# TrevorS/qwen3-tts-rs

Hardware: AMD Instinct MI355X
Metric: acoustic_frames_per_sec (higher is better)
Workload: dtype bf16

## Files before the change

### qwen3_tts_rs_amd/csrc/q3_codec_run.hip

```cpp
#include "q3_engine.h"

namespace {
struct DevCache {
    std::mutex mu;
    std::unordered_multimap<uint64_t, void*> free_blocks;
    std::unordered_map<void*, uint64_t> live;
    size_t cached = 0, cap = 0;
    DevCache() { const char* e = getenv("Q3_DEV_CACHE_MB"); cap = (size_t)(e ? atol(e) : 32768) << 20; }
    static uint64_t key(int dev, size_t bytes) { return ((uint64_t)dev << 48) | (uint64_t)bytes; }
    static size_t size_class(size_t bytes) {
        if (bytes <= 4096) return (bytes + 255) & ~(size_t)255;
        size_t p2 = 1; while ((p2 << 1) <= bytes) p2 <<= 1;
        const size_t step = p2 >> 4;
        return (bytes + step - 1) / step * step;
    }
    hipError_t get(void** p, size_t bytes) {
        bytes = size_class(bytes);
        int dev = 0; (void)hipGetDevice(&dev);
        const uint64_t k = key(dev, bytes);
        {
            std::lock_guard<std::mutex> g(mu);
            auto it = free_blocks.find(k);
            if (it != free_blocks.end()) { *p = it->second; free_blocks.erase(it); cached -= bytes; live[*p] = k; return hipSuccess; }
        }
// ... 86 lines not shown
static thread_local const q3_model* tl_codec_model = nullptr;
static const void* packed_of(const float* w) { return tl_codec_model ? tl_codec_model->pk(w) : nullptr; }
static thread_local int tl_codec_planes = 3;
CodecScope::CodecScope(const q3_model* m) {
    static const int env_planes = [] { const char* e = getenv("Q3_CODEC_PLANES"); const int v = e ? atoi(e) : 0; return (v == 2 || v == 3) ? v : 0; }();
    planes = env_planes ? env_planes : m->codec_planes;
    tl_codec_model = m; tl_codec_planes = planes;
}
CodecScope::~CodecScope() { tl_codec_planes = 3; }
static hipError_t conv1(const float* x, const float* w, const float* b, float* y, int cin, int cout, int L, hipStream_t st,
                        const float* resid = nullptr, const float* scale = nullptr, int act = 0,
                        const float* sa = nullptr, const float* sib = nullptr) {
    ConvArgs a; a.x = x; a.w = w; a.b = b; a.y = y; a.cin = cin; a.cout = cout; a.L = L; a.k = 1; a.dil = 1;
    a.resid = resid; a.scale = scale; a.act = act; a.snake_a = sa; a.snake_b = sib; a.wpk = packed_of(w); a.planes = tl_codec_planes;
    return launch_conv1d(a, st);
}
static hipError_t convk(const float* x, const float* w, const float* b, float* y, int cin, int cout, int L, int k, int dil,
                        hipStream_t st, const float* sa = nullptr, const float* sib = nullptr, int act = 0) {
    ConvArgs a; a.x = x; a.w = w; a.b = b; a.y = y; a.cin = cin; a.cout = cout; a.L = L; a.k = k; a.dil = dil;
    a.snake_a = sa; a.snake_b = sib; a.act = act; a.wpk = packed_of(w); a.planes = tl_codec_planes;
    return launch_conv1d(a, st);
}

static q3_status tap_out(float** taps, int id, const float* dev, size_t n, hipStream_t st) {
    if (taps && taps[id]) { HIPC(hipStreamSynchronize(st)); HIPC(q3_hipMemcpy(taps[id], dev, n * 4, hipMemcpyDeviceToHost)); }
    return Q3_OK;
}
q3_status codec_front_quant(const q3_model* m, CodecWS& ws, int T, hipStream_t st) {
    const q3_config& c = m->cfg;
    const int CD = c.dec_cb_dim, Q = c.dec_q_dim;
    float *A = ws.bufA, *B = ws.bufB;
    float* e1 = A; float* e2 = A + (size_t)CD * T;
    HIPC(launch_rvq_embed(ws.frames, T, m->first_cb, m->rest_cbs_dev, e1, e2, CD, c.dec_cb_size, st));
    HIPC(conv1(e1, m->first_proj, nullptr, B, CD, Q, T, st));
    HIPC(conv1(e2, m->rest_proj, nullptr, B, CD, Q, T, st, B));
    return Q3_OK;
}
q3_status codec_front_preconv(const q3_model* m, const float* x, float* y, int L, hipStream_t st) {
    HIPC(convk(x, m->pre_w, m->pre_b, y, m->cfg.dec_q_dim, m->cfg.dec_latent, L, 3, 1, st));
    return Q3_OK;
}
q3_status codec_front_transformer(const q3_model* m, CodecWS& ws, int T, hipStream_t st, const CodecAttnFn& rope_attn) {
    const q3_config& c = m->cfg;
    const int LAT = c.dec_latent, DH = c.dec_hidden, QD = c.dec_heads * c.dec_head_dim, DI = c.dec_inter;
    float *A = ws.bufA, *B = ws.bufB, *C = ws.bufC, *D = ws.bufD, *E = ws.bufE;
    float* Hd = D;
    HIPC(conv1(C, m->inp_w, m->inp_b, Hd, LAT, DH, T, st));
    float* Nn = E;
    float* q = A; float* k = A + (size_t)QD * T; float* v = A + (size_t)2 * QD * T; float* ao = A + (size_t)3 * QD * T;
    float* g = B; float* u = B + (size_t)DI * T;
    for (int l = 0; l < c.dec_layers; ++l) {
        const DecLayerW& L = m->dl[l];
        HIPC(launch_rmsnorm_c(Hd, L.in_ln, Nn, DH, T, c.dec_eps, st));
        auto adjacent = [&](const float* w0, const float* w1, int cout, int cin) {
            const char* p0 = (const char*)m->pk(w0); const char* p1 = (const char*)m->pk(w1);
            return p0 && p1 && p1 == p0 + packed_conv_w_bytes(cout, cin, 1) && w1 == w0 + (size_t)cout * cin &&
                   cout % 32 == 0 && cin % 16 == 0;
        };
        static const bool no_fuse_qkv = getenv("Q3_CODEC_NO_QKV_FUSE") != nullptr || getenv("Q3_CONV_F32") != nullptr ||
                                        getenv("Q3_CONV_VALU") != nullptr;
        if (!no_fuse_qkv && adjacent(L.q, L.k, QD, DH) && adjacent(L.k, L.v, QD, DH)) {
            HIPC(conv1(Nn, L.q, nullptr, q, DH, 3 * QD, T, st));
        } else {
            HIPC(conv1(Nn, L.q, nullptr, q, DH, QD, T, st));
            HIPC(conv1(Nn, L.k, nullptr, k, DH, QD, T, st));
            HIPC(conv1(Nn, L.v, nullptr, v, DH, QD, T, st));
        }
        Q3C(rope_attn(l, q, k, v, ao));
        HIPC(conv1(ao, L.o, nullptr, Hd, QD, DH, T, st, Hd, L.attn_scale));
        HIPC(launch_rmsnorm_c(Hd, L.post_ln, Nn, DH, T, c.dec_eps, st));
        if (!no_fuse_qkv && adjacent(L.gate, L.up, DI, DH)) {
            HIPC(conv1(Nn, L.gate, nullptr, g, DH, 2 * DI, T, st));
        } else {
            HIPC(conv1(Nn, L.gate, nullptr, g, DH, DI, T, st));
            HIPC(conv1(Nn, L.up, nullptr, u, DH, DI, T, st));
        }
        HIPC(launch_silu_mul(g, u, g, (int64_t)DI * T, st));
        HIPC(conv1(g, L.down, nullptr, Hd, DI, DH, T, st, Hd, L.mlp_scale));
    }
    HIPC(launch_rmsnorm_c(Hd, m->dec_norm, Nn, DH, T, c.dec_eps, st));
    HIPC(conv1(Nn, m->outp_w, m->outp_b, C, DH, LAT, T, st));
    return Q3_OK;
}
q3_status codec_stack_dev(const q3_model* m, CodecWS& ws, float* cur, int L, hipStream_t st, float** taps, const CodecScope& scope) {
    const int NPL = scope.planes;
    const q3_config& c = m->cfg;
    const int LAT = c.dec_latent;
    auto TAP = [&](int id, const float* dev, size_t n) -> q3_status { return tap_out(taps, id, dev, n, st); };
    float *A = ws.bufA, *B = ws.bufB, *C = ws.bufC;
    for (int i = 0; i < 2; ++i) {
        const UpW& U = m->up[i];
        float* upo = (cur == C) ? A : C;
        HIPC(launch_transconv1d_taps(cur, U.tw, U.tb, upo, LAT, LAT, L, U.ratio, 1, nullptr, nullptr, st, nullptr, nullptr, nullptr, m->pk(U.tw), NPL));
        L *= U.ratio;
        float* dw = (upo == A) ? C : A;
        HIPC(launch_dwconv7(upo, U.dww, U.dwb, dw, LAT, L, st));
        float* ln = dw + (size_t)LAT * L;
        HIPC(launch_layernorm_c(dw, U.nw, U.nb, ln, LAT, L, 1e-6f, st));
        HIPC(conv1(ln, U.p1w, U.p1b, B, LAT, 4 * LAT, L, st, nullptr, nullptr, 1));
        HIPC(conv1(B, U.p2w, U.p2b, upo, 4 * LAT, LAT, L, st, upo, U.gamma));
        cur = upo;
        Q3C(TAP(Q3_DEC_UP0 + i, cur, (size_t)LAT * L));
    }
    int Cc = c.dec_dim;
    float* pool4[4] = {A, B, C, ws.bufF};
    auto other = [&](std::initializer_list<const float*> used) -> float* {
        for (float* p : pool4) { bool u = false; for (const float* q : used) if (q == p) u = true; if (!u) return p; }
        return nullptr;
    };
    float* xact = other({cur});
    {
        ConvArgs a; a.x = cur; a.w = m->init_w; a.wpk = m->pk(m->init_w); a.b = m->init_b; a.cin = LAT; a.cout = Cc; a.L = L; a.k = 7; a.dil = 1; a.planes = NPL;
        a.post_a = m->blk[0].a; a.post_ib = m->blk[0].ib;
        if (taps && taps[Q3_DEC_INIT]) { float* raw = other({cur, xact}); a.y = raw; a.y2 = xact; HIPC(launch_conv1d(a, st)); Q3C(TAP(Q3_DEC_INIT, raw, (size_t)Cc * L)); }
        else { a.y = xact; HIPC(launch_conv1d(a, st)); }
    }
    static const int dils[3] = {1, 3, 9};
    for (int b = 0; b < 4; ++b) {
        const DecBlockW& Bk = m->blk[b];
        float* Y = other({xact});
        float* YA = other({xact, Y});
        HIPC(launch_transconv1d_taps(xact, Bk.tw, Bk.tb, Y, Bk.cin, Bk.cout, L, Bk.rate, 2, nullptr, nullptr, st, Bk.res[0].a1, Bk.res[0].ib1, YA, m->pk(Bk.tw), NPL));
        L *= Bk.rate; Cc = Bk.cout;
        float* T2 = other({Y, YA});
        for (int uu = 0; uu < 3; ++uu) {
            const ResUnitW& R = Bk.res[uu];
            const float* nxt_a = uu < 2 ? Bk.res[uu + 1].a1 : (b < 3 ? m->blk[b + 1].a : m->fin_a);
            const float* nxt_ib = uu < 2 ? Bk.res[uu + 1].ib1 : (b < 3 ? m->blk[b + 1].ib : m->fin_ib);
            {
                ResUnitArgs r{};
                r.xa = YA; r.y = Y; r.ya = T2; r.w1pk = m->pk(R.c1w); r.w2pk = m->pk(R.c2w); r.b1 = R.c1b; r.b2 = R.c2b;
                r.mid_a = R.a2; r.mid_ib = R.ib2; r.post_a = nxt_a; r.post_ib = nxt_ib; r.C = Cc; r.L = L; r.dil = dils[uu]; r.planes = NPL;
                const hipError_t e = launch_resunit(r, st);
                if (e == hipSuccess) { float* t = YA; YA = T2; T2 = t; continue; }
                if (e != hipErrorNotSupported) HIPC(e);
            }
            {
                ConvArgs a; a.x = YA; a.w = R.c1w; a.wpk = m->pk(R.c1w); a.b = R.c1b; a.y = T2; a.cin = Cc; a.cout = Cc; a.L = L; a.k = 7; a.dil = dils[uu]; a.planes = NPL;
                a.post_a = R.a2; a.post_ib = R.ib2;
                HIPC(launch_conv1d(a, st));
            }
            {
                ConvArgs a; a.x = T2; a.w = R.c2w; a.wpk = m->pk(R.c2w); a.b = R.c2b; a.y = Y; a.y2 = YA; a.cin = Cc; a.cout = Cc; a.L = L; a.k = 1; a.dil = 1; a.resid = Y; a.planes = NPL;
                if (uu < 2) { a.post_a = Bk.res[uu + 1].a1; a.post_ib = Bk.res[uu + 1].ib1; }
                else if (b < 3) { a.post_a = m->blk[b + 1].a; a.post_ib = m->blk[b + 1].ib; }
                else { a.post_a = m->fin_a; a.post_ib = m->fin_ib; }
                HIPC(launch_conv1d(a, st));
            }
        }
        Q3C(TAP(Q3_DEC_BLK0 + b, Y, (size_t)Cc * L));
        xact = YA;
    }
    HIPC(convk(xact, m->fin_w, m->fin_b, ws.pcm, Cc, 1, L, 7, 1, st, nullptr, nullptr, 2));
    return Q3_OK;
}

q3_status codec_decode_dev(const q3_model* m, CodecWS& ws, int T, hipStream_t st, float** taps, int c0) {
    const q3_config& c = m->cfg;
    const CodecScope scope(m);
    const int Q = c.dec_q_dim, LAT = c.dec_latent;
    float *B = ws.bufB, *C = ws.bufC;
    Q3C(codec_front_quant(m, ws, T, st));
    Q3C(tap_out(taps, Q3_DEC_QUANT, B, (size_t)Q * T, st));
    Q3C(codec_front_preconv(m, B, C, T, st));
    Q3C(tap_out(taps, Q3_DEC_PRECONV, C, (size_t)LAT * T, st));
    const float scale = (float)pow((double)c.dec_head_dim, -0.5);
    Q3C(codec_front_transformer(m, ws, T, st, [&](int, float* q, float* k, float* v, float* ao) -> q3_status {
        HIPC(launch_rope_c(q, k, ws.cs, ws.sn, c.dec_heads, c.dec_head_dim, T, st));
        HIPC(launch_attn_c(q, k, v, ao, c.dec_heads, c.dec_head_dim, T, scale, st));
        return Q3_OK;
    }));
    Q3C(tap_out(taps, Q3_DEC_PRETRANS, C, (size_t)LAT * T, st));
    float* cur = C;
    int L = T;
    if (c0 > 0) {
        HIPC(launch_copy_rows(C + c0, T, ws.bufF, T - c0, LAT, T - c0, st));
        cur = ws.bufF; L = T - c0;
    }
    return codec_stack_dev(m, ws, cur, L, st, taps, scope);
}

extern "C" q3_status q3_decode_codes(q3_model* m, const uint32_t* frames_host, int n_frames, float* pcm_host, float** taps_host) {
    if (!m || !m->finalized) return set_err(Q3_INVALID_ARG, "model not finalized");
    if (n_frames < 0 || (n_frames > 0 && (!frames_host || !pcm_host))) return set_err(Q3_INVALID_ARG, "q3_decode_codes: bad argument");
    if (n_frames == 0) return Q3_OK;
    for (int f = 0; f < n_frames; ++f)
        for (int g = 1; g < 16; ++g)
            if (frames_host[(size_t)f * 16 + g] >= (uint32_t)m->cfg.dec_cb_size)
                return set_err(Q3_INVALID_ARG, "code %u out of range for codebook %d (frame %d)", frames_host[(size_t)f * 16 + g], g, f);
    HIPC(hipSetDevice(m->device));
    CodecWS ws;
    q3_status st = codec_reserve(m, ws, n_frames);
    if (st == Q3_OK) {
        hipError_t e = q3_hipMemcpy(ws.frames, frames_host, (size_t)n_frames * 16 * 4, hipMemcpyHostToDevice);
        if (e != hipSuccess) st = set_err(Q3_HIP_ERROR, "hipMemcpy frames: %s", hipGetErrorString(e));
    }
    if (st == Q3_OK) st = codec_decode_dev(m, ws, n_frames, 0, taps_host);
    if (st == Q3_OK) {
        hipError_t e = q3_hipDeviceSynchronize();
        if (e == hipSuccess) e = q3_hipMemcpy(pcm_host, ws.pcm, (size_t)n_frames * samples_per_frame(m->cfg) * 4, hipMemcpyDeviceToHost);
        if (e != hipSuccess) st = set_err(Q3_HIP_ERROR, "decode: %s", hipGetErrorString(e));
    }
    ws.release();
    return st;
}
```

### qwen3_tts_rs_amd/csrc/q3_engine.h

```cpp
#pragma once
#include "../../include/q3tts.h"
#include "q3_kernels.h"

#include <math.h>
#include <stdarg.h>
#include <stdio.h>
#include <string.h>

#include <algorithm>
#include <atomic>
#include <chrono>
#include <functional>
#include <memory>
#include <string>
#include <thread>
#include <mutex>
#include <unordered_map>
#include <vector>

#include "q3_internal.h"
#include "q3_aql.h"

using namespace q3;
#define Q3_HIDDEN __attribute__((visibility("hidden")))
// ... 225 lines not shown
    void release() {
        dev_free(bufA); dev_free(bufB); dev_free(bufC); dev_free(bufF); dev_free(bufD); dev_free(bufE); dev_free(cs); dev_free(sn); dev_free(frames); dev_free(pcm);
        bufA = bufB = bufC = bufF = bufD = bufE = cs = sn = pcm = nullptr; frames = nullptr; cap_frames = 0; cap_front = 0;
    }
};

struct LmBuf { float *X, *SUM, *QKV, *Q, *ATT, *ACT, *PART; };
struct LmDims { int H, I, nh, nkv, layers; float eps; };

struct BatReq {
    q3_request r{}; std::vector<uint32_t> text, instruct, ref_codes, ref_text; std::vector<float> xvec;
    void own(const q3_request& q, int hidden) {
        r = q;
        text.assign(q.text_ids, q.text_ids + (q.text_ids ? q.n_text : 0));
        instruct.assign(q.instruct_ids, q.instruct_ids + (q.instruct_ids ? q.n_instruct : 0));
        ref_codes.assign(q.ref_codes, q.ref_codes + (q.ref_codes ? (size_t)q.n_ref * 16 : 0));
        ref_text.assign(q.ref_text_ids, q.ref_text_ids + (q.ref_text_ids ? q.n_ref_text : 0));
        if (q.xvector) xvec.assign(q.xvector, q.xvector + hidden);
        fix();
    }
    void fix() {
        r.text_ids = text.empty() ? nullptr : text.data(); r.n_text = (int32_t)text.size();
        r.instruct_ids = instruct.empty() ? nullptr : instruct.data(); r.n_instruct = (int32_t)instruct.size();
        r.ref_codes = ref_codes.empty() ? nullptr : ref_codes.data(); r.n_ref = (int32_t)(ref_codes.size() / 16);
        r.ref_text_ids = ref_text.empty() ? nullptr : ref_text.data(); r.n_ref_text = (int32_t)ref_text.size();
        r.xvector = xvec.empty() ? nullptr : xvec.data();
    }
};
struct SeqInfo {
    q3_request req; std::vector<uint32_t> text, instruct, ref_codes, ref_text; std::vector<float> xvec; bool icl = false;
    int prefill_len = 0, trailing_len = 0, row_base = 0, n_rows = 0, trail_base = 0, pad_row = 0;
    int n_frames = 0; bool done = false;
    int start_run = 0, limit = 0, stream_pos = 0;
    int reused = 0;
    bool idle = false;
    int max_length_req = 0;
    bool opened = false, text_closed = true;
    std::vector<uint32_t> text_all;
    int n_trail = 0, ready = 0x7fffffff, committed = 0;
};

struct ProfAcc { double ms = 0; double bytes = 0; long launches = 0; };
struct ProfShape { int M, N, K, epi, rms, produce, tiled, count; };

struct q3_session {
    q3_model* m = nullptr; int B = 0;
    hipStream_t stream = nullptr; bool owns_stream = true;
    DevPool pool;
    std::vector<SeqInfo> seq;
    q3_options opts{};
    int max_frames = 0, max_seq = 0, prefill_len = 0, n_splits = 1;
    int* limit = nullptr;
    SampleRow* sample_rows = nullptr;
    int row_cap = 0, repl_base = 0;
    LmBuf tb{}, cb{};
    float *LASTH = nullptr, *LOGITS = nullptr, *CP_IN = nullptr, *CP_LOGITS = nullptr;
    float* wide_ws = nullptr; size_t wide_ws_bytes = 0;
    float *kcache = nullptr, *vcache = nullptr, *ckcache = nullptr, *cvcache = nullptr;
    size_t kv_layer_stride = 0, ckv_layer_stride = 0;
    bool paged = false; unsigned long long* kv_table = nullptr; std::vector<std::vector<float*>> kv_rows;
    std::vector<BatReq> ragged;
    bool regrouped = false;
    bool prefix_common = false;
    int kv_overflow_row = -1;
    bool kv_bf16 = false, kv_in_bf16 = false; unsigned long long* kv_conv = nullptr;
    float *rows = nullptr, *embeds = nullptr, *xvec = nullptr; int n_rows_total = 0;
    uint32_t* ids_dev = nullptr; int *tr_dev = nullptr, *ci_dev = nullptr; float *proj_e = nullptr, *proj_h = nullptr;
    uint32_t* ref_codes_dev = nullptr;
    int *trail_base = nullptr, *trail_len = nullptr, *pad_row = nullptr;
    int* text_ready = nullptr;
    uint32_t* app_ids = nullptr; float *app_e = nullptr, *app_h = nullptr, *app_out = nullptr;
    int* flush_buf = nullptr; size_t flush_cap = 0;
    uint32_t* tok = nullptr; uint8_t* seen = nullptr; int *frame_idx = nullptr, *pos = nullptr, *token_count = nullptr;
    float* U = nullptr; uint32_t* codes = nullptr;
    float* logits_hist = nullptr; float* cp_logits_hist = nullptr; bool debug = false;
    bool prefilled = false; int frames_run = 0;
    hipGraphExec_t graph_exec = nullptr; hipGraph_t graph = nullptr;
    q3::AqlProgram* aql = nullptr; int aql_mode = 0; bool aql_tried = false, aql_failed = false;
    bool precapture = false;
    CodecWS cws;
    q3_codec_stream* cstream = nullptr;
    hipStream_t dec_stream = nullptr; hipEvent_t dec_ev = nullptr;
    std::vector<CodecWS> par_ws; std::vector<hipStream_t> par_streams;
    CodecWS seg_ws;
    std::vector<uint32_t> codes_host; bool codes_host_valid = false;
    int stream_pos = 0;
    int stream_mode = 0;
    bool profile = false; ProfAcc prof_linear;
    bool legacy_attn = getenv("Q3_LEGACY_ATTN") != nullptr;
    bool proj_tables = getenv("Q3_NO_PROJ_TABLES") == nullptr;
    bool qkv_tables = getenv("Q3_NO_QKV_TABLES") == nullptr;
    bool ksplit = getenv("Q3_NO_KSPLIT") == nullptr;
    bool cp_attn = getenv("Q3_NO_CP_ATTN") == nullptr;
    bool no_chunk = getenv("Q3_NO_CHUNK") != nullptr;
    std::vector<std::pair<hipEvent_t, hipEvent_t>> prof_events; std::vector<double> prof_event_bytes;
    std::vector<hipEvent_t> prof_pool; size_t prof_pool_next = 0;
    std::vector<ProfShape> prof_shapes;
#ifdef Q3_TRACE
    unsigned long long* trace_buf = nullptr; int trace_node = 0, trace_cap = 0;
    struct TraceMeta { int kind, a, b, c, d, e, f; };
    std::vector<TraceMeta> trace_meta;
    unsigned long long* trace_next(int kind, int a, int b, int c, int d = 0, int e = 0, int f = 0) {
        if (!trace_buf || trace_node >= trace_cap) return nullptr;
        trace_meta.push_back({kind, a, b, c, d, e, f});
        return trace_buf + (size_t)(trace_node++) * TRACE_NODE;
    }
#endif
    ~q3_session();
};


Q3_HIDDEN void model_destroy(q3_model* m);
Q3_HIDDEN void retile_bf16(const uint16_t* src, int N, int K, uint16_t* dst, int mode);
Q3_HIDDEN q3_status codec_reserve(const q3_model* m, CodecWS& ws, int T, int Tf = 0);
Q3_HIDDEN int samples_per_frame(const q3_config& c);
Q3_HIDDEN q3_status codec_decode_dev(const q3_model* m, CodecWS& ws, int T, hipStream_t st, float** taps, int c0 = 0);
struct Q3_HIDDEN CodecScope { int planes; explicit CodecScope(const q3_model* m); ~CodecScope(); CodecScope(const CodecScope&) = delete; };
using CodecAttnFn = std::function<q3_status(int layer, float* q, float* k, float* v, float* ao)>;
Q3_HIDDEN q3_status codec_rope_table(const q3_config& c, int n, float* cs_dev, float* sn_dev);
Q3_HIDDEN q3_status codec_front_quant(const q3_model* m, CodecWS& ws, int T, hipStream_t st);
Q3_HIDDEN q3_status codec_front_preconv(const q3_model* m, const float* x, float* y, int L, hipStream_t st);
Q3_HIDDEN q3_status codec_front_transformer(const q3_model* m, CodecWS& ws, int T, hipStream_t st, const CodecAttnFn& rope_attn);
Q3_HIDDEN q3_status codec_stack_dev(const q3_model* m, CodecWS& ws, float* cur, int L, hipStream_t st, float** taps, const CodecScope& scope);
struct CsPush { int row; int n; int skip; const uint32_t* host; const uint32_t* dev; float* pcm_host; };
Q3_HIDDEN q3_status codec_stream_create(q3_model* m, int rows, int max_frames, hipStream_t st, q3_codec_stream** out, int block_frames = 0,
                                        int max_blocks = 0);
Q3_HIDDEN q3_status codec_stream_push(q3_codec_stream* cs, const std::vector<CsPush>& pushes);
Q3_HIDDEN int codec_stream_pos(const q3_codec_stream* cs, int row);
Q3_HIDDEN void codec_stream_blocks(const q3_codec_stream* cs, int row, int upto, int* held, int* need);
Q3_HIDDEN void codec_stream_reset(q3_codec_stream* cs, int row);
Q3_HIDDEN hipError_t sync_frames(q3_session* s);
Q3_HIDDEN q3_status kv_reserve_row(q3_session* s, int b, int n_pos);
Q3_HIDDEN q3_status kv_reserve_frames(q3_session* s, int frames);
Q3_HIDDEN void kv_release_row(q3_session* s, int b);
Q3_HIDDEN LmDims talker_dims(const q3_config& c);
Q3_HIDDEN LmDims cp_dims(const q3_config& c);
Q3_HIDDEN q3_status talker_step(q3_session* s, const int* pos_dev, int pos_static, bool with_head, int rows_per_seq = 1,
                                const int* text_ready = nullptr);
Q3_HIDDEN SampleRow sample_row(const q3_options& o);
Q3_HIDDEN void request_shape(const q3_request& r, int* prefill_len, int* limit);
Q3_HIDDEN long row_worst_units(int prefill_len, int limit, bool bf16);
Q3_HIDDEN q3_request idle_request(int chunk_frames);
Q3_HIDDEN q3_status session_create(q3_model* m, const q3_request* reqs, int batch, int frame_budget, int prompt_budget, q3_session** out,
                                   hipStream_t borrow = nullptr);
Q3_HIDDEN q3_status lm_layer(q3_session* s, const LmDims& d, const LayerW& w, LmBuf& b, float* kc, float* vc, int max_seq,
                             const int* pos_dev, int pos_static, int n_splits, int rows_per_seq = 1, bool skip_qkv = false,
                             const CpGatherArgs* fold = nullptr, int paged_layer = -1);
struct TextPiece { int b; const uint32_t* ids; int n; bool last; };
Q3_HIDDEN q3_status session_text_enable(q3_session* s);
Q3_HIDDEN q3_status session_append_many(q3_session* s, const std::vector<TextPiece>& pieces);
Q3_HIDDEN int session_row_remaining(const q3_session* s, int b);
Q3_HIDDEN int session_row_committed(const q3_session* s, int b);
Q3_HIDDEN q3_status transplant_row(q3_session* s, int b, q3_session* side, int j, int limit);
Q3_HIDDEN q3_status transplant_check(q3_session* s, q3_session* side, int j, int limit_req, int* limit_out);
```

### qwen3_tts_rs_amd/csrc/q3_session.hip

```cpp
#include "q3_engine.h"
#include "q3_prefix_cache.h"

hipError_t sync_frames(q3_session* s) {
    if (s->aql) {
        std::string why;
        if (!q3::aql_wait(s->aql, &why)) { s->aql_failed = true; set_err(Q3_HIP_ERROR, "AQL frame submission: %s", why.c_str()); return hipErrorUnknown; }
    }
    return hipStreamSynchronize(s->stream);
}

static hipError_t run_linear(q3_session* s, const LinArgs& a_in) {
    LinArgs a = a_in;
    a.ws = s->wide_ws; a.ws_bytes = s->wide_ws_bytes;
#ifdef Q3_TRACE
    a.trace = s->trace_next(0, a.M, a.N, a.K, a.epi, a.norm_w ? 1 : 0, a.tiled);
#endif
    if (!s->profile) return launch_linear(a, s->stream);
    hipEvent_t e0, e1;
    if (s->prof_pool_next + 2 <= s->prof_pool.size()) { e0 = s->prof_pool[s->prof_pool_next++]; e1 = s->prof_pool[s->prof_pool_next++]; }
    else {
        hipError_t e = hipEventCreate(&e0); if (e != hipSuccess) return e;
        e = hipEventCreate(&e1); if (e != hipSuccess) return e;
        s->prof_pool.push_back(e0); s->prof_pool.push_back(e1); s->prof_pool_next = s->prof_pool.size();
    }
// ... 501 lines not shown
    HIPC(alloc_lm(s->tb, talker_dims(c), s->n_splits));
    HIPC(alloc_lm(s->cb, cp_dims(c), 1));
    if (B > 16) {
        size_t need = 0;
        auto upd = [&](int N, int K, int epi) { if (N % 128 == 0 && K % 128 == 0) { const size_t b = gemm_wide_ws_bytes(B, N, K, epi); if (b > need) need = b; } };
        const int QDt = c.n_heads * HEAD_DIM, KDt = c.n_kv_heads * HEAD_DIM, QDc = c.cp_heads * HEAD_DIM, KDc = c.cp_kv_heads * HEAD_DIM;
        upd(QDt + 2 * KDt, H, EPI_NONE); upd(H, QDt, EPI_RESID); upd(c.inter, H, EPI_SWIGLU); upd(H, c.inter, EPI_RESID); upd(c.codec_vocab, H, EPI_NONE);
        upd(QDc + 2 * KDc, c.cp_hidden, EPI_NONE); upd(c.cp_hidden, QDc, EPI_RESID); upd(c.cp_inter, c.cp_hidden, EPI_SWIGLU); upd(c.cp_hidden, c.cp_inter, EPI_RESID);
        upd(c.cp_vocab, c.cp_hidden, EPI_NONE); upd(c.cp_hidden, H, EPI_NONE);
        if (need) { HIPC(s->pool.alloc(&s->wide_ws, need / 4)); s->wide_ws_bytes = need; }
    }
    HIPC(s->pool.alloc(&s->LASTH, (size_t)B * H));
    HIPC(s->pool.alloc(&s->LOGITS, (size_t)B * c.codec_vocab));
    HIPC(s->pool.alloc(&s->CP_IN, (size_t)(B > 16 ? up16(B) : 16) * H));
    HIPC(s->pool.alloc(&s->CP_LOGITS, (size_t)15 * B * c.cp_vocab));
    s->kv_layer_stride = (size_t)B * c.n_kv_heads * s->max_seq * HEAD_DIM;
    {
        const char* e = getenv("Q3_KV_CONTIGUOUS");
        s->paged = !(e && atoi(e) != 0);
        if (s->paged) {
            if (s->max_seq > KV_MAX_PAGES * KV_PAGE_POS) return set_err(Q3_KV_OVERFLOW, "sequence length %d exceeds a row's page table (%d)", s->max_seq, KV_MAX_PAGES * KV_PAGE_POS);
            HIPC(s->pool.alloc(&s->kv_table, (size_t)B * KV_MAX_PAGES));
            HIPC(s->pool.alloc(&s->kv_conv, (size_t)2 * B * KV_MAX_PAGES));
            s->kv_rows.resize((size_t)B);
            for (auto& r : s->kv_rows) r.reserve(KV_MAX_PAGES);
        } else {
            HIPC(s->pool.alloc(&s->kcache, s->kv_layer_stride * c.n_layers));
            HIPC(s->pool.alloc(&s->vcache, s->kv_layer_stride * c.n_layers));
        }
    }
    s->ckv_layer_stride = (size_t)B * c.cp_kv_heads * (c.n_groups + 1) * HEAD_DIM;
    HIPC(s->pool.alloc(&s->ckcache, 2 * s->ckv_layer_stride * c.cp_layers + 64));
    s->cvcache = s->ckcache + s->ckv_layer_stride * c.cp_layers + 64;
    HIPC(s->pool.alloc(&s->rows, ((size_t)rows + (size_t)B * s->row_cap) * H));
    HIPC(s->pool.alloc(&s->limit, B));
    HIPC(s->pool.alloc(&s->sample_rows, B));
    {
        std::vector<int> lim(B); std::vector<SampleRow> sr(B);
        for (int b = 0; b < B; ++b) { lim[b] = s->seq[b].limit; sr[b] = sample_row(s->seq[b].req.opts); }
        HIPC(q3_hipMemcpy(s->limit, lim.data(), B * 4, hipMemcpyHostToDevice));
        HIPC(q3_hipMemcpy(s->sample_rows, sr.data(), B * sizeof(SampleRow), hipMemcpyHostToDevice));
    }
    HIPC(s->pool.alloc(&s->embeds, (size_t)B * s->prefill_len * H));
    HIPC(s->pool.alloc(&s->xvec, (size_t)B * H));
    HIPC(s->pool.alloc(&s->ids_dev, (size_t)rows)); HIPC(s->pool.alloc(&s->tr_dev, (size_t)B * s->prefill_len)); HIPC(s->pool.alloc(&s->ci_dev, (size_t)B * s->prefill_len));
    HIPC(s->pool.alloc(&s->proj_e, (size_t)rows * c.text_dim)); HIPC(s->pool.alloc(&s->proj_h, (size_t)rows * c.text_dim));
    HIPC(s->pool.alloc(&s->trail_base, B)); HIPC(s->pool.alloc(&s->trail_len, B)); HIPC(s->pool.alloc(&s->pad_row, B));
    HIPC(s->pool.alloc(&s->tok, B)); HIPC(s->pool.alloc(&s->seen, (size_t)B * c.codec_vocab));
    HIPC(s->pool.alloc(&s->frame_idx, B)); HIPC(s->pool.alloc(&s->pos, B)); HIPC(s->pool.alloc(&s->token_count, B));
    HIPC(s->pool.alloc(&s->U, (size_t)B * (s->max_frames + 2)));
    HIPC(s->pool.alloc(&s->codes, (size_t)B * s->max_frames * 16));
    std::vector<float> U((size_t)B * (s->max_frames + 2), 0.0f);
    for (int b = 0; b < B; ++b) {
        uint64_t st;
        const q3_options& o = reqs[b].opts;
        uint64_t seed = o.seed;
        if (!o.has_seed) seed = (uint64_t)std::chrono::high_resolution_clock::now().time_since_epoch().count() + 0x9E37ULL * b;
        q3_rng_seed(seed, &st);
        for (int i = 0; i <= s->max_frames; ++i) U[(size_t)b * (s->max_frames + 2) + i] = q3_rng_next(&st);
    }
    HIPC(q3_hipMemcpy(s->U, U.data(), U.size() * 4, hipMemcpyHostToDevice));
    HIPC(s->pool.settle());
    s->pool.lazy = false;
    *out = s.release();
    return Q3_OK;
}

q3_session::~q3_session() {
    if (!m) return;
    (void)hipSetDevice(m->device);
    if (stream) (void)hipStreamSynchronize(stream);
    if (dec_stream) (void)hipStreamSynchronize(dec_stream);
    for (auto st : par_streams) (void)hipStreamSynchronize(st);
    if (aql) q3::aql_program_destroy(aql);
    for (int b = 0; b < (int)kv_rows.size(); ++b) kv_release_row(this, b);
    if (graph_exec) (void)hipGraphExecDestroy(graph_exec);
    if (graph) (void)hipGraphDestroy(graph);
    for (auto& ev : prof_pool) (void)hipEventDestroy(ev);
    for (auto st : par_streams) (void)hipStreamDestroy(st);
    if (cstream) q3_codec_stream_free(cstream);
    cws.release(); seg_ws.release();
    for (auto& w : par_ws) w.release();
    if (dec_ev) (void)hipEventDestroy(dec_ev);
    if (dec_stream) (void)hipStreamDestroy(dec_stream);
    if (stream && owns_stream) {
        std::lock_guard<std::mutex> g(m->stream_mu);
        if (m->idle_streams.size() < 16) { m->idle_streams.push_back(stream); stream = nullptr; }
    }
    if (stream && owns_stream) (void)hipStreamDestroy(stream);
    pool.release_all();
    if (m->refs.fetch_sub(1) == 1) model_destroy(m);
}

extern "C" void q3_session_free(q3_session* s) { delete s; }

extern "C" q3_status q3_session_set_kv_dtype(q3_session* s, int dtype) {
    if (!s) return set_err(Q3_INVALID_ARG, "null session");
    if (s->prefilled) return set_err(Q3_INVALID_ARG, "q3_session_set_kv_dtype must be called before prefill");
    if (dtype != Q3_DTYPE_F32 && dtype != Q3_DTYPE_BF16) return set_err(Q3_INVALID_ARG, "q3_session_set_kv_dtype: unknown dtype %d", dtype);
    if (dtype == Q3_DTYPE_BF16 && !s->paged) return set_err(Q3_UNSUPPORTED, "bf16 K/V needs the paged cache (Q3_KV_CONTIGUOUS is set)");
    s->kv_bf16 = dtype == Q3_DTYPE_BF16;
    return Q3_OK;
}

extern "C" q3_status q3_session_set_debug(q3_session* s, int capture) {
    if (!s) return set_err(Q3_INVALID_ARG, "null session");
    if (s->prefilled) return set_err(Q3_INVALID_ARG, "set_debug must be called before prefill");
    if (capture && s->text_ready) return set_err(Q3_UNSUPPORTED, "set_debug: the session has open text rows");
    s->debug = capture != 0;
    if (s->debug && !s->logits_hist) {
        const q3_config& c = s->m->cfg;
        HIPC(hipSetDevice(s->m->device));
        HIPC(s->pool.alloc(&s->logits_hist, (size_t)s->B * (s->max_frames + 1) * c.codec_vocab));
        HIPC(s->pool.alloc(&s->cp_logits_hist, (size_t)s->max_frames * 15 * s->B * c.cp_vocab));
    }
    return Q3_OK;
}
extern "C" q3_status q3_session_set_profile(q3_session* s, int enable) {
    if (!s) return set_err(Q3_INVALID_ARG, "null session");
    if (enable && s->text_ready) return set_err(Q3_UNSUPPORTED, "set_profile: the session has open text rows");
    s->profile = enable != 0;
    return Q3_OK;
}
extern "C" q3_status q3_session_stream(q3_session* s, void** stream) {
    if (!s || !stream) return set_err(Q3_INVALID_ARG, "null argument");
    *stream = (void*)s->stream;
    return Q3_OK;
}
extern "C" q3_status q3_session_prefill_len(q3_session* s, int b, int* prefill_len, int* trailing_len) {
    if (!s || b < 0 || b >= s->B) return set_err(Q3_INVALID_ARG, "bad sequence index");
    if (!s->ragged.empty()) {
        int S = 0, L = 0; request_shape(s->ragged[(size_t)b].r, &S, &L);
        if (prefill_len) *prefill_len = S;
        if (trailing_len) *trailing_len = -1;
        return Q3_OK;
    }
    if (prefill_len) *prefill_len = s->seq[b].prefill_len;
    if (trailing_len) *trailing_len = s->seq[b].trailing_len;
    return Q3_OK;
}

static q3_status text_project(q3_session* s, const uint32_t* ids_dev, int n, float* out_rows) {
    const q3_model* m = s->m; const q3_config& c = m->cfg;
    const int TD = c.text_dim, H = c.hidden;
    if (n > s->n_rows_total) return set_err(Q3_INVALID_ARG, "text_project: %d rows exceed the session's %d", n, s->n_rows_total);
    float *e = s->proj_e, *h = s->proj_h;
    q3_status st = Q3_OK;
    hipError_t er = launch_gather_rows_bf16(m->text_emb, ids_dev, e, n, TD, s->stream);
    if (er == hipSuccess && n >= 48 && TD % 64 == 0 && H % 64 == 0 && !s->no_chunk) {
        GemmArgs g1; g1.W = m->fc1w.t1; g1.x = e; g1.ldx = TD; g1.bias = m->fc1b; g1.y = h; g1.ldy = TD;
        g1.M = n; g1.N = TD; g1.K = TD; g1.Kpad = (TD + 31) / 32 * 32; g1.epi = EPI_SILU;
        er = launch_lm_gemm(g1, s->stream);
        if (er == hipSuccess) {
            GemmArgs g2; g2.W = m->fc2w.t1; g2.x = h; g2.ldx = TD; g2.bias = m->fc2b; g2.y = out_rows; g2.ldy = H;
            g2.M = n; g2.N = H; g2.K = TD; g2.Kpad = (TD + 31) / 32 * 32; g2.epi = EPI_NONE;
            er = launch_lm_gemm(g2, s->stream);
        }
    } else
    for (int r0 = 0; r0 < n && er == hipSuccess; r0 += 8) {
        const int M = (n - r0) < 8 ? (n - r0) : 8;
        LinArgs a;
        a.N = TD; a.K = TD; set_w(a, m->fc1w, M, TD, TD); a.x = e + (size_t)r0 * TD; a.ldx = TD; a.bias = m->fc1b; a.y = h + (size_t)r0 * TD; a.ldy = TD; a.M = M; a.epi = EPI_SILU;
        er = launch_linear(a, s->stream);
        if (er != hipSuccess) break;
        LinArgs b2;
        b2.N = H; b2.K = TD; set_w(b2, m->fc2w, M, H, TD); b2.x = h + (size_t)r0 * TD; b2.ldx = TD; b2.bias = m->fc2b; b2.y = out_rows + (size_t)r0 * H; b2.ldy = H; b2.M = M; b2.epi = EPI_NONE;
// ... 865 lines not shown
        n_samples[b] = (size_t)a * spf;
        if (a <= 0) continue;
        if (s->stream_mode == 1 && !q.icl) {
            if (!s->cstream) Q3C(codec_stream_create(s->m, s->B, s->max_frames, s->stream, &s->cstream));
            if (codec_stream_pos(s->cstream, b) > q.stream_pos) codec_stream_reset(s->cstream, b);
            const int sp = codec_stream_pos(s->cstream, b);
            pushes.push_back({b, q.stream_pos + a - sp, q.stream_pos - sp, nullptr, s->codes + ((size_t)b * s->max_frames + sp) * 16,
                              pcm_host ? pcm_host[b] : nullptr});
        } else {
            Q3C(chunk_decode_row(s, b, a, pcm_host ? pcm_host[b] : nullptr, cap ? cap[b] : 0, nullptr));
        }
    }
    if (!pushes.empty()) Q3C(codec_stream_push(s->cstream, pushes));
    for (int b = 0; b < s->B; ++b) {
        SeqInfo& q = s->seq[b];
        q.stream_pos += avail[(size_t)b];
        done[b] = held[(size_t)b] ? 0 : (avail[(size_t)b] <= 0 || (q.done && q.stream_pos >= q.n_frames)) ? 1 : 0;
    }
    return Q3_OK;
}

extern "C" q3_status q3_session_frames(q3_session* s, int b, int* n_frames, int* done) {
    if (!s || b < 0 || b >= s->B) return set_err(Q3_INVALID_ARG, "bad sequence index");
    HIPC(hipSetDevice(s->m->device));
    Q3C(refresh_codes(s));
    if (n_frames) *n_frames = s->seq[b].n_frames;
    if (done) *done = s->seq[b].done ? 1 : 0;
    return Q3_OK;
}

extern "C" q3_status q3_session_codes(q3_session* s, int b, uint32_t* codes_host, int cap_frames, int* n_frames) {
    if (!s || b < 0 || b >= s->B) return set_err(Q3_INVALID_ARG, "bad sequence index");
    HIPC(hipSetDevice(s->m->device));
    Q3C(refresh_codes(s));
    const int n = s->seq[b].n_frames;
    if (n_frames) *n_frames = n;
    if (codes_host) {
        if (cap_frames < n) return set_err(Q3_INVALID_ARG, "codes buffer too small (%d < %d frames)", cap_frames, n);
        memcpy(codes_host, &s->codes_host[(size_t)b * s->max_frames * 16], (size_t)n * 16 * 4);
    }
    return Q3_OK;
}

static q3_status decode_range_on(q3_session* s, int b, int f0, int f1, hipStream_t st, float* pcm_host, size_t cap, size_t* n_samples) {
    const int T = f1 - f0, spf = samples_per_frame(s->m->cfg);
    if (n_samples) *n_samples = (size_t)T * spf;
    if (T == 0) return Q3_OK;
    Q3C(codec_reserve(s->m, s->cws, T));
    HIPC(hipMemcpyAsync(s->cws.frames, s->codes + ((size_t)b * s->max_frames + f0) * 16, (size_t)T * 16 * 4, hipMemcpyDeviceToDevice, st));
    Q3C(codec_decode_dev(s->m, s->cws, T, st, nullptr));
    HIPC(hipStreamSynchronize(st));
    if (pcm_host) {
        if (cap < (size_t)T * spf) return set_err(Q3_INVALID_ARG, "pcm buffer too small");
        HIPC(q3_hipMemcpy(pcm_host, s->cws.pcm, (size_t)T * spf * 4, hipMemcpyDeviceToHost));
    }
    return Q3_OK;
}

extern "C" q3_status q3_session_decode(q3_session* s, int b, int f0, int f1, float* pcm_host, size_t cap, size_t* n_samples) {
    if (!s || b < 0 || b >= s->B) return set_err(Q3_INVALID_ARG, "bad sequence index");
    HIPC(hipSetDevice(s->m->device));
    Q3C(refresh_codes(s));
    if (f0 < 0 || f1 < f0 || f1 > s->seq[b].n_frames) return set_err(Q3_INVALID_ARG, "bad frame range [%d,%d) of %d", f0, f1, s->seq[b].n_frames);
    const int T = f1 - f0, spf = samples_per_frame(s->m->cfg);
    const SeqInfo& q = s->seq[b];
    if (!q.ref_codes.empty() && s->prefilled && f0 == 0 && f1 == q.n_frames) {
        const int n_ref = (int)(q.ref_codes.size() / 16), total = n_ref + T;
        const size_t all = (size_t)total * spf, cut = (size_t)n_ref * all / (size_t)(total > 0 ? total : 1);
        if (n_samples) *n_samples = all - cut;
        Q3C(codec_reserve(s->m, s->cws, total));
        HIPC(hipMemcpyAsync(s->cws.frames, q.ref_codes.data(), (size_t)n_ref * 16 * 4, hipMemcpyHostToDevice, s->stream));
        if (T > 0) HIPC(hipMemcpyAsync(s->cws.frames + (size_t)n_ref * 16, s->codes + (size_t)b * s->max_frames * 16, (size_t)T * 16 * 4, hipMemcpyDeviceToDevice, s->stream));
        Q3C(codec_decode_dev(s->m, s->cws, total, s->stream, nullptr));
        HIPC(sync_frames(s));
        if (pcm_host) {
            if (cap < all - cut) return set_err(Q3_INVALID_ARG, "pcm buffer too small");
            HIPC(q3_hipMemcpy(pcm_host, s->cws.pcm + cut, (all - cut) * 4, hipMemcpyDeviceToHost));
        }
        return Q3_OK;
    }
    return decode_range_on(s, b, f0, f1, s->stream, pcm_host, cap, n_samples);
}

extern "C" q3_status q3_session_run(q3_session* s, int use_graph, float** pcm_host, const size_t* cap, size_t* n_samples, q3_timing* timing) {
    if (!s) return set_err(Q3_INVALID_ARG, "null session");
    if (any_open_text(s)) return set_err(Q3_UNSUPPORTED, "q3_session_run: a row's text is still open (q3_session_append_text with last != 0 closes it; or drive the session with q3_session_generate)");
    using clk = std::chrono::steady_clock;
    auto ms = [](clk::time_point a, clk::time_point b) { return std::chrono::duration<double, std::milli>(b - a).count(); };
    const auto t0 = clk::now();
    s->precapture = use_graph != 0;
    Q3C(q3_session_prefill(s));
    const auto t1 = clk::now();
    const int overlap_env = [] { const char* e = getenv("Q3_DECODE_OVERLAP"); return e ? atoi(e) : 0; }();
    static const int seg_env = [] { const char* e = getenv("Q3_DECODE_SEG"); const int v = e ? atoi(e) : 128; return v < 16 ? 16 : v; }();
    bool overlap = overlap_env != 0 && !s->debug && !s->profile && s->max_frames > seg_env;
    for (auto& q : s->seq) if (!q.ref_codes.empty()) overlap = false;
    const int spf = samples_per_frame(s->m->cfg);
    if (!overlap) {
        Q3C(q3_session_generate(s, s->max_frames, use_graph));
        Q3C(refresh_codes(s));
        const auto t2 = clk::now();
        int total = 0;
        static const int conc = [] { const char* e = getenv("Q3_DECODE_PAIRS"); const int v = e ? atoi(e) : 2; return v < 1 ? 1 : (v > 8 ? 8 : v); }();
        bool any_icl = false;
        for (auto& q : s->seq) any_icl = any_icl || !q.ref_codes.empty();
        if (conc > 1 && s->B > 1 && !any_icl) {
            while ((int)s->par_ws.size() < conc - 1) {
                s->par_ws.emplace_back();
                hipStream_t st = nullptr;
                HIPC(hipStreamCreateWithFlags(&st, hipStreamNonBlocking));
                s->par_streams.push_back(st);
            }
            auto ws_of = [&](int k) -> CodecWS& { return k == 0 ? s->cws : s->par_ws[(size_t)k - 1]; };
            auto st_of = [&](int k) { return k == 0 ? s->stream : s->par_streams[(size_t)k - 1]; };
            if (pcm_host)
                for (int b = 0; b < s->B; ++b)
                    if (pcm_host[b] && s->seq[b].n_frames && (!cap || cap[b] < (size_t)s->seq[b].n_frames * spf)) return set_err(Q3_INVALID_ARG, "pcm buffer too small");
            for (int b0 = 0; b0 < s->B; b0 += conc) {
                const int nb = (s->B - b0) < conc ? (s->B - b0) : conc;
                for (int k = 0; k < nb; ++k) {
                    const int b = b0 + k, T = s->seq[b].n_frames;
                    if (n_samples) n_samples[b] = (size_t)T * spf;
                    total += T;
                    if (T == 0) continue;
                    Q3C(codec_reserve(s->m, ws_of(k), T));
                    HIPC(hipMemcpyAsync(ws_of(k).frames, s->codes + (size_t)b * s->max_frames * 16, (size_t)T * 16 * 4, hipMemcpyDeviceToDevice, st_of(k)));
                    Q3C(codec_decode_dev(s->m, ws_of(k), T, st_of(k), nullptr));
                    if (pcm_host && pcm_host[b])
                        HIPC(hipMemcpyAsync(pcm_host[b], ws_of(k).pcm, (size_t)T * spf * 4, hipMemcpyDeviceToHost, st_of(k)));
                }
                for (int k = 0; k < nb; ++k) HIPC(hipStreamSynchronize(st_of(k)));
            }
        } else
        for (int b = 0; b < s->B; ++b) {
            size_t n = 0;
            Q3C(q3_session_decode(s, b, 0, s->seq[b].n_frames, pcm_host ? pcm_host[b] : nullptr, cap ? cap[b] : 0, &n));
            if (n_samples) n_samples[b] = n;
            total += s->seq[b].n_frames;
        }
        const auto t3 = clk::now();
        if (timing) { timing->prefill_ms = ms(t0, t1); timing->generation_ms = ms(t1, t2); timing->decode_ms = ms(t2, t3); timing->generation_frames = total; }
        return Q3_OK;
    }
    HIPC(hipSetDevice(s->m->device));
    static const int cus = [] { const char* e = getenv("Q3_DECODE_CUS"); const int v = e ? atoi(e) : 0; return v <= 0 ? 0 : (v < 8 ? 8 : (v > 248 ? 248 : v & ~7)); }();
    if (!s->dec_stream) {
        if (cus) {
            uint32_t mask[8] = {0, 0, 0, 0, 0, 0, 0, 0};
            for (int i = 256 - cus; i < 256; ++i) mask[i >> 5] |= 1u << (i & 31);
            HIPC(hipExtStreamCreateWithCUMask(&s->dec_stream, 8, mask));
        } else {
            int least = 0, greatest = 0;
            HIPC(hipDeviceGetStreamPriorityRange(&least, &greatest));
            HIPC(hipStreamCreateWithPriority(&s->dec_stream, hipStreamNonBlocking, least));
        }
    }
    Q3C(codec_reserve(s->m, s->seg_ws, seg_env + CODEC_CTX_FRAMES, s->max_frames));
    struct Split {
        q3::AqlProgram* p = nullptr;
        void release() { if (p) { std::string why; q3::aql_restrict_cus(p, 0, &why); p = nullptr; } }
        ~Split() { release(); }
    } split;
    if (cus && s->aql && !s->aql_failed) { std::string why; if (q3::aql_restrict_cus(s->aql, 256 - cus, &why)) split.p = s->aql; }
    std::vector<int> dec_pos((size_t)s->B, 0);
    std::thread worker; q3_status wst = Q3_OK; std::string werr;
    auto join = [&]() -> q3_status {
        if (worker.joinable()) worker.join();
        if (wst != Q3_OK) return set_err(wst, "%s", werr.c_str());
        return Q3_OK;
    };
    struct Job { int b, a, e; };
    auto seg_enqueue = [s, spf, pcm_host, cap](const Job& j, CodecWS& ws, hipStream_t st) -> q3_status {
        const int c0 = j.a > CODEC_CTX_FRAMES ? j.a - CODEC_CTX_FRAMES : 0;
        if (pcm_host && pcm_host[j.b] && (!cap || cap[j.b] < (size_t)j.e * spf)) return set_err(Q3_INVALID_ARG, "pcm buffer too small");
        HIPC(hipMemcpyAsync(ws.frames, s->codes + (size_t)j.b * s->max_frames * 16, (size_t)j.e * 16 * 4, hipMemcpyDeviceToDevice, st));
        Q3C(codec_decode_dev(s->m, ws, j.e, st, nullptr, c0));
        if (pcm_host && pcm_host[j.b])
            HIPC(hipMemcpyAsync(pcm_host[j.b] + (size_t)j.a * spf, ws.pcm + (size_t)(j.a - c0) * spf, (size_t)(j.e - j.a) * spf * 4, hipMemcpyDeviceToHost, st));
        return Q3_OK;
    };
    auto collect = [&](bool final_pass) {
        std::vector<Job> jobs;
        for (int b = 0; b < s->B; ++b) {
            const SeqInfo& q = s->seq[b];
            const int e = (q.done || final_pass) ? q.n_frames : (q.n_frames < s->frames_run ? q.n_frames : s->frames_run);
            if (e > dec_pos[(size_t)b] && (final_pass || q.done || e - dec_pos[(size_t)b] >= 16)) {
                for (int a = dec_pos[(size_t)b]; a < e; a += seg_env) jobs.push_back({b, a, a + seg_env < e ? a + seg_env : e});
                dec_pos[(size_t)b] = e;
            }
// ... 177 lines not shown
```

Baseline: 2844.

## Pipeline codec decode across rows with front/back split on two streams

Splits codec decode into a front stage (quantizer, preconv, transformer, optionally upsampling) and a back stage (conv stack), then runs rows in a two-stream software pipeline. The front of row k+1 runs on a side stream while the stack of row k runs on the main stream, and PCM device-to-host copies are also issued on the side stream. Events and double-buffered workspaces coordinate the two streams. The aim is to overlap the small-kernel front half with the heavy conv stack and hide copy latency. It replaces the default paired-concurrency path whenever host PCM buffers are given, and adds cross-stream synchronization that could serialize if the stages are unbalanced.

```diff
diff --git a/qwen3_tts_rs_amd/csrc/q3_codec_run.hip b/qwen3_tts_rs_amd/csrc/q3_codec_run.hip
--- a/qwen3_tts_rs_amd/csrc/q3_codec_run.hip
+++ b/qwen3_tts_rs_amd/csrc/q3_codec_run.hip
@@ -192,12 +192,11 @@
     HIPC(conv1(Nn, m->outp_w, m->outp_b, C, DH, LAT, T, st));
     return Q3_OK;
 }
-q3_status codec_stack_dev(const q3_model* m, CodecWS& ws, float* cur, int L, hipStream_t st, float** taps, const CodecScope& scope) {
-    const int NPL = scope.planes;
-    const q3_config& c = m->cfg;
-    const int LAT = c.dec_latent;
+q3_status codec_up_dev(const q3_model* m, CodecWS& ws, float** cur_io, int* L_io, hipStream_t st, float** taps, const CodecScope& scope) {
+    const int NPL = scope.planes, LAT = m->cfg.dec_latent;
     auto TAP = [&](int id, const float* dev, size_t n) -> q3_status { return tap_out(taps, id, dev, n, st); };
     float *A = ws.bufA, *B = ws.bufB, *C = ws.bufC;
+    float* cur = *cur_io; int L = *L_io;
     for (int i = 0; i < 2; ++i) {
         const UpW& U = m->up[i];
         float* upo = (cur == C) ? A : C;
@@ -212,6 +211,16 @@
         cur = upo;
         Q3C(TAP(Q3_DEC_UP0 + i, cur, (size_t)LAT * L));
     }
+    *cur_io = cur; *L_io = L;
+    return Q3_OK;
+}
+q3_status codec_stack_dev(const q3_model* m, CodecWS& ws, float* cur, int L, hipStream_t st, float** taps, const CodecScope& scope, bool up_done) {
+    if (!up_done) Q3C(codec_up_dev(m, ws, &cur, &L, st, taps, scope));
+    const int NPL = scope.planes;
+    const q3_config& c = m->cfg;
+    const int LAT = c.dec_latent;
+    auto TAP = [&](int id, const float* dev, size_t n) -> q3_status { return tap_out(taps, id, dev, n, st); };
+    float *A = ws.bufA, *B = ws.bufB, *C = ws.bufC;
     int Cc = c.dec_dim;
     float* pool4[4] = {A, B, C, ws.bufF};
     auto other = [&](std::initializer_list<const float*> used) -> float* {
@@ -266,6 +275,11 @@
 }
 
 q3_status codec_decode_dev(const q3_model* m, CodecWS& ws, int T, hipStream_t st, float** taps, int c0) {
+    CodecMid mid;
+    Q3C(codec_front_dev(m, ws, T, st, taps, c0, false, &mid));
+    return codec_back_dev(m, ws, mid, st, taps);
+}
+q3_status codec_front_dev(const q3_model* m, CodecWS& ws, int T, hipStream_t st, float** taps, int c0, bool with_up, CodecMid* mid) {
     const q3_config& c = m->cfg;
     const CodecScope scope(m);
     const int Q = c.dec_q_dim, LAT = c.dec_latent;
@@ -281,13 +295,17 @@
         return Q3_OK;
     }));
     Q3C(tap_out(taps, Q3_DEC_PRETRANS, C, (size_t)LAT * T, st));
-    float* cur = C;
-    int L = T;
+    mid->cur = C; mid->L = T; mid->up_done = false;
     if (c0 > 0) {
         HIPC(launch_copy_rows(C + c0, T, ws.bufF, T - c0, LAT, T - c0, st));
-        cur = ws.bufF; L = T - c0;
-    }
-    return codec_stack_dev(m, ws, cur, L, st, taps, scope);
+        mid->cur = ws.bufF; mid->L = T - c0;
+    }
+    if (with_up) { Q3C(codec_up_dev(m, ws, &mid->cur, &mid->L, st, taps, scope)); mid->up_done = true; }
+    return Q3_OK;
+}
+q3_status codec_back_dev(const q3_model* m, CodecWS& ws, const CodecMid& mid, hipStream_t st, float** taps) {
+    const CodecScope scope(m);
+    return codec_stack_dev(m, ws, mid.cur, mid.L, st, taps, scope, mid.up_done);
 }
 
 extern "C" q3_status q3_decode_codes(q3_model* m, const uint32_t* frames_host, int n_frames, float* pcm_host, float** taps_host) {
diff --git a/qwen3_tts_rs_amd/csrc/q3_engine.h b/qwen3_tts_rs_amd/csrc/q3_engine.h
--- a/qwen3_tts_rs_amd/csrc/q3_engine.h
+++ b/qwen3_tts_rs_amd/csrc/q3_engine.h
@@ -331,6 +331,7 @@
     q3_codec_stream* cstream = nullptr;
     hipStream_t dec_stream = nullptr; hipEvent_t dec_ev = nullptr;
     std::vector<CodecWS> par_ws; std::vector<hipStream_t> par_streams;
+    hipEvent_t pipe_front_ev[2] = {nullptr, nullptr}, pipe_stack_ev[2] = {nullptr, nullptr}, pipe_copy_ev[2] = {nullptr, nullptr};
     CodecWS seg_ws;
     std::vector<uint32_t> codes_host; bool codes_host_valid = false;
     int stream_pos = 0;
@@ -370,7 +371,11 @@
 Q3_HIDDEN q3_status codec_front_quant(const q3_model* m, CodecWS& ws, int T, hipStream_t st);
 Q3_HIDDEN q3_status codec_front_preconv(const q3_model* m, const float* x, float* y, int L, hipStream_t st);
 Q3_HIDDEN q3_status codec_front_transformer(const q3_model* m, CodecWS& ws, int T, hipStream_t st, const CodecAttnFn& rope_attn);
-Q3_HIDDEN q3_status codec_stack_dev(const q3_model* m, CodecWS& ws, float* cur, int L, hipStream_t st, float** taps, const CodecScope& scope);
+Q3_HIDDEN q3_status codec_up_dev(const q3_model* m, CodecWS& ws, float** cur_io, int* L_io, hipStream_t st, float** taps, const CodecScope& scope);
+Q3_HIDDEN q3_status codec_stack_dev(const q3_model* m, CodecWS& ws, float* cur, int L, hipStream_t st, float** taps, const CodecScope& scope, bool up_done = false);
+struct CodecMid { float* cur = nullptr; int L = 0; bool up_done = false; };
+Q3_HIDDEN q3_status codec_front_dev(const q3_model* m, CodecWS& ws, int T, hipStream_t st, float** taps, int c0, bool with_up, CodecMid* mid);
+Q3_HIDDEN q3_status codec_back_dev(const q3_model* m, CodecWS& ws, const CodecMid& mid, hipStream_t st, float** taps);
 struct CsPush { int row; int n; int skip; const uint32_t* host; const uint32_t* dev; float* pcm_host; };
 Q3_HIDDEN q3_status codec_stream_create(q3_model* m, int rows, int max_frames, hipStream_t st, q3_codec_stream** out, int block_frames = 0,
                                         int max_blocks = 0);
diff --git a/qwen3_tts_rs_amd/csrc/q3_session.hip b/qwen3_tts_rs_amd/csrc/q3_session.hip
--- a/qwen3_tts_rs_amd/csrc/q3_session.hip
+++ b/qwen3_tts_rs_amd/csrc/q3_session.hip
@@ -607,6 +607,8 @@
     cws.release(); seg_ws.release();
     for (auto& w : par_ws) w.release();
     if (dec_ev) (void)hipEventDestroy(dec_ev);
+    for (int i = 0; i < 2; ++i)
+        for (hipEvent_t ev : {pipe_front_ev[i], pipe_stack_ev[i], pipe_copy_ev[i]}) if (ev) (void)hipEventDestroy(ev);
     if (dec_stream) (void)hipStreamDestroy(dec_stream);
     if (stream && owns_stream) {
         std::lock_guard<std::mutex> g(m->stream_mu);
@@ -1638,6 +1640,83 @@
     return decode_range_on(s, b, f0, f1, s->stream, pcm_host, cap, n_samples);
 }
 
+static q3_status decode_pipeline(q3_session* s, float** pcm_host, int mode) {
+    static const bool with_up = [] { const char* e = getenv("Q3_DECODE_PIPE_UP"); return e ? atoi(e) != 0 : true; }();
+    const int spf = samples_per_frame(s->m->cfg);
+    std::vector<int> rows;
+    int Tmax = 0;
+    for (int b = 0; b < s->B; ++b)
+        if (s->seq[b].n_frames > 0) { rows.push_back(b); if (s->seq[b].n_frames > Tmax) Tmax = s->seq[b].n_frames; }
+    if (rows.empty()) return Q3_OK;
+    if (s->par_ws.empty()) {
+        hipStream_t st = nullptr;
+        HIPC(hipStreamCreateWithFlags(&st, hipStreamNonBlocking));
+        s->par_ws.emplace_back(); s->par_streams.push_back(st);
+    }
+    for (int i = 0; i < 2; ++i)
+        for (hipEvent_t* ev : {&s->pipe_front_ev[i], &s->pipe_stack_ev[i], &s->pipe_copy_ev[i]})
+            if (!*ev) HIPC(hipEventCreateWithFlags(ev, hipEventDisableTiming));
+    Q3C(codec_reserve(s->m, s->cws, Tmax));
+    Q3C(codec_reserve(s->m, s->par_ws[0], Tmax));
+    const hipStream_t main_st = s->stream, side_st = s->par_streams[0];
+    auto ws_of = [&](int k) -> CodecWS& { return (k & 1) ? s->par_ws[0] : s->cws; };
+    const int n = (int)rows.size();
+    CodecMid mid[2];
+    auto codes_in = [&](int k, hipStream_t st) -> q3_status {
+        const int b = rows[(size_t)k];
+        HIPC(hipMemcpyAsync(ws_of(k).frames, s->codes + (size_t)b * s->max_frames * 16, (size_t)s->seq[b].n_frames * 16 * 4, hipMemcpyDeviceToDevice, st));
+        return Q3_OK;
+    };
+    auto pcm_out = [&](int k, hipStream_t st) -> q3_status {
+        const int b = rows[(size_t)k];
+        HIPC(hipMemcpyAsync(pcm_host[b], ws_of(k).pcm, (size_t)s->seq[b].n_frames * spf * 4, hipMemcpyDeviceToHost, st));
+        return Q3_OK;
+    };
+    auto front = [&](int k) -> q3_status {
+        const int w = k & 1;
+        if (k >= 2) HIPC(hipStreamWaitEvent(side_st, s->pipe_stack_ev[w], 0));
+        Q3C(codes_in(k, side_st));
+        Q3C(codec_front_dev(s->m, ws_of(k), s->seq[rows[(size_t)k]].n_frames, side_st, nullptr, 0, with_up, &mid[w]));
+        HIPC(hipEventRecord(s->pipe_front_ev[w], side_st));
+        return Q3_OK;
+    };
+    auto stack = [&](int k) -> q3_status {
+        const int w = k & 1, b = rows[(size_t)k];
+        HIPC(hipStreamWaitEvent(main_st, s->pipe_front_ev[w], 0));
+        if (k >= 2 && pcm_host[rows[(size_t)k - 2]]) HIPC(hipStreamWaitEvent(main_st, s->pipe_copy_ev[w], 0));
+        Q3C(codec_back_dev(s->m, ws_of(k), mid[w], main_st, nullptr));
+        HIPC(hipEventRecord(s->pipe_stack_ev[w], main_st));
+        if (pcm_host[b]) {
+            HIPC(hipStreamWaitEvent(side_st, s->pipe_stack_ev[w], 0));
+            Q3C(pcm_out(k, side_st));
+            HIPC(hipEventRecord(s->pipe_copy_ev[w], side_st));
+        }
+        return Q3_OK;
+    };
+    auto enqueue = [&]() -> q3_status {
+        if (mode == 2) {
+            for (int k = 0; k < n; ++k) {
+                const hipStream_t st = (k & 1) ? side_st : main_st;
+                Q3C(codes_in(k, st));
+                Q3C(codec_decode_dev(s->m, ws_of(k), s->seq[rows[(size_t)k]].n_frames, st, nullptr));
+                if (pcm_host[rows[(size_t)k]]) Q3C(pcm_out(k, st));
+            }
+            return Q3_OK;
+        }
+        Q3C(front(0));
+        for (int k = 0; k < n; ++k) {
+            if (k + 1 < n) Q3C(front(k + 1));
+            Q3C(stack(k));
+        }
+        return Q3_OK;
+    };
+    const q3_status st = enqueue();
+    const hipError_t e1 = hipStreamSynchronize(main_st), e2 = hipStreamSynchronize(side_st);
+    if (st != Q3_OK) return st;
+    HIPC(e1); HIPC(e2);
+    return Q3_OK;
+}
+
 extern "C" q3_status q3_session_run(q3_session* s, int use_graph, float** pcm_host, const size_t* cap, size_t* n_samples, q3_timing* timing) {
     if (!s) return set_err(Q3_INVALID_ARG, "null session");
     if (any_open_text(s)) return set_err(Q3_UNSUPPORTED, "q3_session_run: a row's text is still open (q3_session_append_text with last != 0 closes it; or drive the session with q3_session_generate)");
@@ -1660,7 +1739,16 @@
         static const int conc = [] { const char* e = getenv("Q3_DECODE_PAIRS"); const int v = e ? atoi(e) : 2; return v < 1 ? 1 : (v > 8 ? 8 : v); }();
         bool any_icl = false;
         for (auto& q : s->seq) any_icl = any_icl || !q.ref_codes.empty();
-        if (conc > 1 && s->B > 1 && !any_icl) {
+        const int pipe_env = [] { const char* e = getenv("Q3_DECODE_PIPE"); return e ? atoi(e) : 1; }();
+        if (pipe_env != 0 && s->B > 1 && !any_icl && pcm_host) {
+            for (int b = 0; b < s->B; ++b) {
+                const int T = s->seq[b].n_frames;
+                if (pcm_host[b] && T && (!cap || cap[b] < (size_t)T * spf)) return set_err(Q3_INVALID_ARG, "pcm buffer too small");
+                if (n_samples) n_samples[b] = (size_t)T * spf;
+                total += T;
+            }
+            Q3C(decode_pipeline(s, pcm_host, pipe_env));
+        } else if (conc > 1 && s->B > 1 && !any_icl) {
             while ((int)s->par_ws.size() < conc - 1) {
                 s->par_ws.emplace_back();
                 hipStream_t st = nullptr;
```

New measurement: 2848, median of 6. About the same (+0.1%).
